# LouisRouss/DiffuLab

Hardware: AMD Instinct MI355X
Metric: train images/sec/node (DiT-S/2 flow-matching, 256x256 latents) (higher is better)
Workload: dtype bf16

## Files before the change

diffulab_amd/csrc/attention.hip:

```cpp
#include "common.h"
#include "attn_paths.h"

static std::atomic<int> g_last_attn_path{DL_ATTN_PATH_NONE};
void dl_note_attn_path(int path) { g_last_attn_path.store(path, std::memory_order_relaxed); }
extern "C" __attribute__((visibility("default"))) int dl_lab_last_attn_path() { return g_last_attn_path.load(std::memory_order_relaxed); }

typedef __attribute__((address_space(3))) void lds_void_t;
typedef const __attribute__((address_space(1))) void glb_void_t;

#define DH 64
#define ROWB 128
#define LOG2E 1.4426950408889634f
#define LN2 0.6931471805599453f

__device__ __forceinline__ int swz8(int row) {
  const int v = (row >> 1) & 7;
  return ((v & 1) << 2) | (v >> 1);
}
__device__ __forceinline__ int tile_off(int row, int slot) { return row * ROWB + ((slot ^ swz8(row)) << 4); }

__device__ __forceinline__ void tile_dma(const bf16_t* __restrict__ g, int64_t pitch, char* tile, int nrows, int wave,
                                         int nwaves, int lane) {
  const int nchunk = nrows >> 3;
  for (int c = wave; c < nchunk; c += nwaves) {
// ... 576 lines not shown
    f32x16_t s[2];
#pragma unroll
    for (int t = 0; t < 2; ++t) {
#pragma unroll
      for (int r = 0; r < 16; ++r) s[t][r] = 0.f;
#pragma unroll
      for (int ks = 0; ks < 4; ++ks) s[t] = MFMA(frag_rows(kt, kb + t * 32 + (lane & 31), ks, hi), qf[ks], s[t]);
    }
    float mx = -INFINITY;
#pragma unroll
    for (int t = 0; t < 2; ++t)
#pragma unroll
      for (int r = 0; r < 16; ++r) {
        s[t][r] *= c;
        mx = fmaxf(mx, s[t][r]);
      }
    mx = fmaxf(mx, __shfl_xor(mx, 32, 64));
    const float m_new = fmaxf(m_run, mx);
    const float alpha = fast_exp2(m_run - m_new);
    m_run = m_new;
    float ps = 0.f;
    float p[2][16];
#pragma unroll
    for (int t = 0; t < 2; ++t)
#pragma unroll
      for (int r = 0; r < 16; ++r) {
        p[t][r] = fast_exp2(s[t][r] - m_new);
        ps += p[t][r];
      }
    l_run = l_run * alpha + ps;
#pragma unroll
    for (int r = 0; r < 16; ++r) {
      o[0][r] *= alpha;
      o[1][r] *= alpha;
    }
#pragma unroll
    for (int t = 0; t < 2; ++t)
#pragma unroll
      for (int kg2 = 0; kg2 < 2; ++kg2) {
        const bf16x8_t pf = pack_frag(&p[t][kg2 * 8]);
        const int rbase = kb + t * 32 + kg2 * 16;
        o[0] = MFMA(frag_cols(vt, rbase, 0, lane), pf, o[0]);
        o[1] = MFMA(frag_cols(vt, rbase, 32, lane), pf, o[1]);
      }
  }
  const float l_tot = l_run + __shfl_xor(l_run, 32, 64);
  const float inv = 1.0f / l_tot;
  store_rows64(out + ((int64_t)b * N + qrow) * (H * DH) + h * DH, o, inv, hi);
  if (hi == 0) lse[(int64_t)bh * N + qrow] = (m_run + log2f(l_tot)) * LN2;
}

static int g_attn_pipe = 1;
extern "C" __attribute__((visibility("default"))) void dl_lab_set_attn_pipe(int mode) { g_attn_pipe = mode; }
static int attn_fwd_pipe_on() { return g_attn_pipe & 1; }
#define PIPE_N 256
__global__ __launch_bounds__(512) void attn_fwd_qkn_pipe_k(const bf16_t* __restrict__ qkv, bf16_t* __restrict__ out, float* __restrict__ lse,
                                                           int H, int items, float scale, QkNorm qn) {
  constexpr int N = PIPE_N;
  extern __shared__ __attribute__((aligned(16))) char smem[];
  const int lane = threadIdx.x & 63, hi = lane >> 5, l31 = lane & 31;
  const int wave = __builtin_amdgcn_readfirstlane(threadIdx.x >> 6);
  const int per = (items + (int)gridDim.x - 1) / (int)gridDim.x;
  const int it0 = blockIdx.x * per, it1 = it0 + per < items ? it0 + per : items;
  if (it0 >= it1) return;
  const int D = H * DH, half = qn.rot >> 1;
  const int qrow = wave * 32 + l31;
  f32x4_t qc[4], qs[4];
#pragma unroll
  for (int ks = 0; ks < 4; ++ks) {
    const int d0 = ks * 16 + hi * 8;
    if (d0 < qn.rot) {
      qc[ks] = *(const f32x4_t*)(qn.cs + (int64_t)qrow * half + (d0 >> 1));
      qs[ks] = *(const f32x4_t*)(qn.sn + (int64_t)qrow * half + (d0 >> 1));
    } else {
      qc[ks] = qs[ks] = f32x4_t{0.f, 0.f, 0.f, 0.f};
    }
  }
  int ro[4];
#pragma unroll
  for (int ks = 0; ks < 4; ++ks) ro[ks] = tile_off(l31, ks * 2 + hi);
  int co[2][2];
  {
    const int li = lane & 15, g = lane >> 4;
#pragma unroll
    for (int cb = 0; cb < 2; ++cb)
#pragma unroll
      for (int hh = 0; hh < 2; ++hh) {
        const int col = cb * 32 + (g & 1) * 16 + (li & 3) * 4, r = (g >> 1) * 4 + (li >> 2) + 8 * hh;
        co[cb][hh] = r * ROWB + (((col >> 3) ^ swz8(r)) << 4) + (col & 7) * 2;
      }
  }
  const float c = scale * LOG2E;
  float* sq_l = (float*)(smem + 4 * N * ROWB);
  float* sk_l = sq_l + D;
  for (int i = threadIdx.x; i < D; i += blockDim.x) {
    sq_l[i] = qn.sq[i];
    sk_l[i] = qn.sk[i];
  }

  u32x4_t qraw[4];
  float ssq_q, ssq_k;
  u32x4_t opk[4];
  float lse_pend = 0.f;
  auto store_pending = [&](int item) {
    const int b = item / H, h = item - b * H;
    bf16_t* rowp = out + ((int64_t)b * N + qrow) * (H * DH) + h * DH;
#pragma unroll
    for (int dt = 0; dt < 2; ++dt)
#pragma unroll
      for (int gp = 0; gp < 2; ++gp) *(u32x4_t*)(rowp + dt * 32 + 16 * gp + 8 * hi) = opk[dt * 2 + gp];
    if (hi == 0) lse[(int64_t)item * N + qrow] = lse_pend;
  };
  auto issue_tiles = [&](int item, int buf) {
    const int b = item / H, h = item - b * H;
    const bf16_t* base = qkv + (int64_t)b * N * qn.pitch + h * DH;
    char* kt = smem + buf * (2 * N * ROWB);
    tile_dma(base + D, qn.pitch, kt, N, wave, 8, lane);
    tile_dma(base + 2 * D, qn.pitch, kt + N * ROWB, N, wave, 8, lane);
  };
  auto issue_regs = [&](int item) {
    const int b = item / H, h = item - b * H;
    const bf16_t* base = qkv + (int64_t)b * N * qn.pitch + h * DH;
#pragma unroll
    for (int ks = 0; ks < 4; ++ks) qraw[ks] = *(const u32x4_t*)(base + (int64_t)qrow * qn.pitch + ks * 16 + hi * 8);
    const float2 sq2 = *(const float2*)(qn.ssq + ((int64_t)b * N + qrow) * 2);
    ssq_q = sq2.x;
    ssq_k = sq2.y;
  };
  issue_regs(it0);
  issue_tiles(it0, 0);

  for (int it = it0; it < it1; ++it) {
    const int buf = (it - it0) & 1;
    char* kt = smem + buf * (2 * N * ROWB);
    char* vt = kt + N * ROWB;
    const int b = it / H, h = it - b * H, bh = it;
    const int64_t tok = (int64_t)b * N + qrow;
    asm volatile("s_waitcnt vmcnt(0)" ::: "memory");
    __syncthreads();
    const float rq = rsqrtf(ssq_q * qn.inv_d + qn.eps);
    bf16x8_t qf[4];
#pragma unroll
    for (int ks = 0; ks < 4; ++ks) {
      const int d0 = ks * 16 + hi * 8;
      const u32x4_t t = qk_xform8(qraw[ks], rq, sq_l + h * DH + d0, (const float*)&qc[ks], (const float*)&qs[ks], d0 < qn.rot);
      qf[ks] = __builtin_bit_cast(bf16x8_t, t);
      if (qn.qo) *(u32x4_t*)(qn.qo + ((int64_t)bh * N + qrow) * DH + d0) = t;
    }
    if (qn.rrms && h == 0 && hi == 0) qn.rrms[tok * 2] = rq;
    const float rk = rsqrtf(ssq_k * qn.inv_d + qn.eps);
#pragma unroll
    for (int ks = 0; ks < 4; ++ks) {
      const int d0 = ks * 16 + hi * 8;
      char* p = kt + wave * 32 * ROWB + ro[ks];
      const u32x4_t t = qk_xform8(*(const u32x4_t*)p, rk, sk_l + h * DH + d0, (const float*)&qc[ks], (const float*)&qs[ks], d0 < qn.rot);
      *(u32x4_t*)p = t;
      if (qn.ko) *(u32x4_t*)(qn.ko + ((int64_t)bh * N + qrow) * DH + d0) = t;
    }
    if (qn.rrms && h == 0 && hi == 0) qn.rrms[tok * 2 + 1] = rk;
    if (it > it0) store_pending(it - 1);
    if (it + 1 < it1) issue_regs(it + 1);
    __syncthreads();
    if (it + 1 < it1) issue_tiles(it + 1, buf ^ 1);

    f32x16_t o[2];
#pragma unroll
    for (int r = 0; r < 16; ++r) o[0][r] = o[1][r] = 0.f;
    float m_run = -INFINITY, l_run = 0.f;
#pragma unroll 1
    for (int kb = 0; kb < N; kb += 64) {
      union {
        s16x4_t h[2];
        bf16x8_t v;
      } vf[2][2][2];
#pragma unroll
      for (int t = 0; t < 2; ++t)
#pragma unroll
        for (int kg2 = 0; kg2 < 2; ++kg2)
#pragma unroll
          for (int cb = 0; cb < 2; ++cb) {
            const char* pb = vt + (kb + t * 32 + kg2 * 16) * ROWB;
            vf[t][kg2][cb].h[0] = attn_lds_tr16(pb + co[cb][0]);
            vf[t][kg2][cb].h[1] = attn_lds_tr16(pb + co[cb][1]);
          }
      f32x16_t s[2];
#pragma unroll
      for (int t = 0; t < 2; ++t) {
#pragma unroll
        for (int r = 0; r < 16; ++r) s[t][r] = 0.f;
#pragma unroll
        for (int ks = 0; ks < 4; ++ks) s[t] = MFMA(*(const bf16x8_t*)(kt + (kb + t * 32) * ROWB + ro[ks]), qf[ks], s[t]);
      }
      float mx = -INFINITY;
#pragma unroll
      for (int t = 0; t < 2; ++t)
#pragma unroll
        for (int r = 0; r < 16; ++r) {
          s[t][r] *= c;
          mx = fmaxf(mx, s[t][r]);
        }
      mx = fmaxf(mx, __shfl_xor(mx, 32, 64));
      const float m_new = fmaxf(m_run, mx);
      const float alpha = fast_exp2(m_run - m_new);
      m_run = m_new;
      float ps = 0.f;
      float p[2][16];
#pragma unroll
      for (int t = 0; t < 2; ++t)
#pragma unroll
        for (int r = 0; r < 16; ++r) {
          p[t][r] = fast_exp2(s[t][r] - m_new);
          ps += p[t][r];
        }
      l_run = l_run * alpha + ps;
#pragma unroll
      for (int r = 0; r < 16; ++r) {
        o[0][r] *= alpha;
        o[1][r] *= alpha;
      }
      asm volatile("s_waitcnt lgkmcnt(0)" ::: "memory");
#pragma unroll
      for (int t = 0; t < 2; ++t)
#pragma unroll
        for (int kg2 = 0; kg2 < 2; ++kg2)
#pragma unroll
          for (int cb = 0; cb < 2; ++cb) asm volatile("" : "+v"(vf[t][kg2][cb].v));
#pragma unroll
      for (int t = 0; t < 2; ++t)
#pragma unroll
        for (int kg2 = 0; kg2 < 2; ++kg2) {
          const bf16x8_t pf = pack_frag(&p[t][kg2 * 8]);
          o[0] = MFMA(vf[t][kg2][0].v, pf, o[0]);
          o[1] = MFMA(vf[t][kg2][1].v, pf, o[1]);
        }
    }
    const float l_tot = l_run + __shfl_xor(l_run, 32, 64);
    const float inv = 1.0f / l_tot;
    pack_rows64(opk, o, inv);
    lse_pend = (m_run + log2f(l_tot)) * LN2;
  }
  store_pending(it1 - 1);
}

extern "C" int dl_attn_fwd_qkn(const void* qkv, const float* ssq, const float* scale_q, const float* scale_k, const float* cos,
                               const float* sin, float eps, int64_t rot, void* q_out, void* k_out, float* rrms, void* out, float* lse,
                               int64_t B, int64_t H, int64_t N, int64_t dh, float scale, dl_stream_t stream) {
  DL_CHECK_ARG(qkv && ssq && scale_q && scale_k && out && lse && B > 0 && H > 0, "dl_attn_fwd_qkn: null operand");
  DL_CHECK_ARG((q_out && k_out && rrms) || (!q_out && !k_out && !rrms), "dl_attn_fwd_qkn: q_out, k_out and rrms are kept together (training) or not at all");
  DL_CHECK_ARG(rot == 0 || (cos && sin), "dl_attn_fwd_qkn: rot > 0 needs the cos / sin tables");
  DL_CHECK_ARG(dh == DH && rot % 8 == 0 && rot <= DH, "dl_attn_fwd_qkn: head_dim 64, rot %% 8 == 0 (dh=%lld rot=%lld)", (long long)dh,
               (long long)rot);
  DL_CHECK_ARG(N % 64 == 0 && N >= 64 && N <= 256, "dl_attn_fwd_qkn: N=%lld must be a multiple of 64 up to 256", (long long)N);
  DL_CHECK_ARG((((uintptr_t)qkv | (uintptr_t)q_out | (uintptr_t)k_out | (uintptr_t)out | (uintptr_t)scale_q | (uintptr_t)scale_k |
                 (uintptr_t)cos | (uintptr_t)sin) & 15) == 0, "dl_attn_fwd_qkn: 16-byte alignment");
  const int lds = (int)(2 * N * ROWB);
  static DevOnce once;
  (void)dev_cus(once, [] { (void)hipFuncSetAttribute((const void*)attn_fwd_qkn_k, hipFuncAttributeMaxDynamicSharedMemorySize, 2 * 256 * ROWB); });
  const int64_t D = H * DH;
  QkNorm qn{ssq, scale_q, scale_k, cos, sin, (bf16_t*)q_out, (bf16_t*)k_out, rrms, 1.0f / (float)D, eps, (int)rot, (int)(3 * D)};
  const int cus = dev_cus(once, [] {});
  if (N == PIPE_N && D <= 2048 && B * H >= 3 * (int64_t)cus && attn_fwd_pipe_on()) {
    static DevOnce once2;
    (void)dev_cus(once2, [] { (void)hipFuncSetAttribute((const void*)attn_fwd_qkn_pipe_k, hipFuncAttributeMaxDynamicSharedMemorySize, 4 * PIPE_N * ROWB + 8 * 2048); });
    const int items = (int)(B * H);
    const int per = (items + cus - 1) / cus, grid = (items + per - 1) / per;
    dl_note_attn_path(ATTN_FWD_QKN_PIPE);
    hipLaunchKernelGGL(attn_fwd_qkn_pipe_k, grid, 512, 4 * PIPE_N * ROWB + 8 * (int)D, (hipStream_t)stream, (const bf16_t*)qkv, (bf16_t*)out, lse, (int)H,
                       items, scale, qn);
    DL_LAUNCH_CHECK();
    return DL_OK;
  }
  dl_note_attn_path(ATTN_FWD_QKN_CHAIN);
  hipLaunchKernelGGL(attn_fwd_qkn_k, (int)(B * H), (int)(N / 32) * 64, lds, (hipStream_t)stream, (const bf16_t*)qkv, (bf16_t*)out, lse, (int)H,
                     (int)N, scale, qn);
  DL_LAUNCH_CHECK();
  return DL_OK;
}

__device__ __forceinline__ bf16x8_t frag_rows_g(const bf16_t* __restrict__ g, int64_t pitch, int row, int ks, int hi) {
  return *(const bf16x8_t*)(g + (int64_t)row * pitch + (ks * 2 + hi) * 8);
}

__global__ __launch_bounds__(256, 2) void attn_bwd_k(const bf16_t* __restrict__ q, const bf16_t* __restrict__ k,
                                                     const bf16_t* __restrict__ v, const bf16_t* __restrict__ out,
                                                     const bf16_t* __restrict__ dout, const float* __restrict__ lse,
                                                     bf16_t* __restrict__ dq, bf16_t* __restrict__ dk,
                                                     bf16_t* __restrict__ dv, int H, int N, float scale, HeadLayout vl,
                                                     HeadLayout dvl, HeadLayout dql) {
  extern __shared__ __attribute__((aligned(16))) char smem[];
  char* ta = smem;
  char* tb = ta + N * ROWB;
  float* lse2 = (float*)(tb + N * ROWB);
  float* delta = lse2 + N;
  const int lane = threadIdx.x & 63, hi = lane >> 5;
  const int wave = __builtin_amdgcn_readfirstlane(threadIdx.x >> 6), nwaves = blockDim.x >> 6;
  const int bh = blockIdx.x, b = bh / H, h = bh - b * H;
  const int64_t hoff = (int64_t)bh * N * DH;
  const int64_t tok_pitch = (int64_t)H * DH;
  const bf16_t* og = out + (int64_t)b * N * tok_pitch + h * DH;
  const bf16_t* dog = dout + (int64_t)b * N * tok_pitch + h * DH;
  tile_dma(k + hoff, DH, ta, N, wave, nwaves, lane);
  const bf16_t* vg = v + b * vl.bs + h * vl.hs;
  tile_dma(vg, vl.pitch, tb, N, wave, nwaves, lane);
  asm volatile("s_waitcnt vmcnt(0)" ::: "memory");
  __syncthreads();

  const float c = scale * LOG2E;

  for (int ob = 0; ob < 2; ++ob) {
    const int own = (wave * 2 + ob) * 32;
    bf16x8_t qf[4], dof[4];
#pragma unroll
    for (int ks = 0; ks < 4; ++ks) {
      qf[ks] = frag_rows_g(q + hoff, DH, own + (lane & 31), ks, hi);
      dof[ks] = frag_rows_g(dog, tok_pitch, own + (lane & 31), ks, hi);
    }
    float my_delta = 0.f;
#pragma unroll
    for (int ks = 0; ks < 4; ++ks) {
      const bf16x8_t of = frag_rows_g(og, tok_pitch, own + (lane & 31), ks, hi);
#pragma unroll
      for (int e = 0; e < 8; ++e) my_delta += (float)of[e] * (float)dof[ks][e];
    }
    my_delta += __shfl_xor(my_delta, 32, 64);
    const float my_lse = lse[(int64_t)bh * N + own + (lane & 31)] * LOG2E;
    if (hi == 0) {
      delta[own + (lane & 31)] = my_delta;
      lse2[own + (lane & 31)] = my_lse;
    }
    f32x16_t dqa[2];
#pragma unroll
    for (int r = 0; r < 16; ++r) dqa[0][r] = dqa[1][r] = 0.f;
    auto scores = [&](int kb, f32x16_t& st, f32x16_t& dpt) {
#pragma unroll
      for (int r = 0; r < 16; ++r) st[r] = dpt[r] = 0.f;
#pragma unroll
      for (int ks = 0; ks < 4; ++ks) {
        st = MFMA(frag_rows(ta, kb + (lane & 31), ks, hi), qf[ks], st);
        dpt = MFMA(frag_rows(tb, kb + (lane & 31), ks, hi), dof[ks], dpt);
      }
    };
    auto step = [&](int kb, f32x16_t& st, f32x16_t& dpt, f32x16_t& stn, f32x16_t& dptn) {
      if (kb + 32 < N) scores(kb + 32, stn, dptn);
      float ds[16];
#pragma unroll
      for (int r = 0; r < 16; ++r) {
        const float p = fast_exp2(st[r] * c - my_lse);
        ds[r] = p * (dpt[r] - my_delta);
      }
#pragma unroll
      for (int kg2 = 0; kg2 < 2; ++kg2) {
        const bf16x8_t df = pack_frag(&ds[kg2 * 8]);
        dqa[0] = MFMA(frag_cols(ta, kb + kg2 * 16, 0, lane), df, dqa[0]);
        dqa[1] = MFMA(frag_cols(ta, kb + kg2 * 16, 32, lane), df, dqa[1]);
      }
    };
    f32x16_t s0, d0, s1, d1;
    scores(0, s0, d0);
    for (int kb = 0; kb < N; kb += 64) {
      step(kb, s0, d0, s1, d1);
      step(kb + 32, s1, d1, s0, d0);
    }
    store_rows64(dq + b * dql.bs + h * dql.hs + (int64_t)(own + (lane & 31)) * dql.pitch, dqa, scale, hi);
  }

  __syncthreads();
  tile_dma(q + hoff, DH, ta, N, wave, nwaves, lane);
  tile_dma(dog, tok_pitch, tb, N, wave, nwaves, lane);
  asm volatile("s_waitcnt vmcnt(0)" ::: "memory");
  __syncthreads();

  for (int ob = 0; ob < 2; ++ob) {
    const int own = (wave * 2 + ob) * 32;
    bf16x8_t kf[4], vf[4];
#pragma unroll
    for (int ks = 0; ks < 4; ++ks) {
      kf[ks] = frag_rows_g(k + hoff, DH, own + (lane & 31), ks, hi);
      vf[ks] = frag_rows_g(vg, vl.pitch, own + (lane & 31), ks, hi);
    }
    f32x16_t dka[2], dva[2];
#pragma unroll
    for (int r = 0; r < 16; ++r) dka[0][r] = dka[1][r] = dva[0][r] = dva[1][r] = 0.f;
    auto scores_t = [&](int qb, f32x16_t& s) {
#pragma unroll
      for (int r = 0; r < 16; ++r) s[r] = 0.f;
#pragma unroll
      for (int ks = 0; ks < 4; ++ks) s = MFMA(frag_rows(ta, qb + (lane & 31), ks, hi), kf[ks], s);
    };
    auto step_t = [&](int qb, f32x16_t& s, f32x16_t& sn) {
      f32x16_t dp;
#pragma unroll
      for (int r = 0; r < 16; ++r) dp[r] = 0.f;
#pragma unroll
      for (int ks = 0; ks < 4; ++ks) dp = MFMA(frag_rows(tb, qb + (lane & 31), ks, hi), vf[ks], dp);
      if (qb + 32 < N) scores_t(qb + 32, sn);
      float p[16], ds[16];
#pragma unroll
      for (int g4 = 0; g4 < 4; ++g4) {
        const f32x4_t l4 = *(const f32x4_t*)(lse2 + qb + g4 * 8 + hi * 4);
        const f32x4_t d4 = *(const f32x4_t*)(delta + qb + g4 * 8 + hi * 4);
#pragma unroll
        for (int e = 0; e < 4; ++e) {
          const int r = g4 * 4 + e;
          p[r] = fast_exp2(s[r] * c - l4[e]);
          ds[r] = p[r] * (dp[r] - d4[e]);
        }
      }
#pragma unroll
      for (int kg2 = 0; kg2 < 2; ++kg2) {
        const bf16x8_t pf = pack_frag(&p[kg2 * 8]);
        const bf16x8_t df = pack_frag(&ds[kg2 * 8]);
        const int rbase = qb + kg2 * 16;
        dva[0] = MFMA(frag_cols(tb, rbase, 0, lane), pf, dva[0]);
        dva[1] = MFMA(frag_cols(tb, rbase, 32, lane), pf, dva[1]);
        dka[0] = MFMA(frag_cols(ta, rbase, 0, lane), df, dka[0]);
        dka[1] = MFMA(frag_cols(ta, rbase, 32, lane), df, dka[1]);
      }
    };
    f32x16_t s0, s1;
    scores_t(0, s0);
    for (int qb = 0; qb < N; qb += 32) {
      step_t(qb, s0, s1);
      s0 = s1;
    }
    store_rows64(dk + b * dql.bs + h * dql.hs + (int64_t)(own + (lane & 31)) * dql.pitch, dka, scale, hi);
    store_rows64(dv + b * dvl.bs + h * dvl.hs + (int64_t)(own + (lane & 31)) * dvl.pitch, dva, 1.0f, hi);
  }
}

__global__ __launch_bounds__(256, 2) void attn_bwd_tiled_k(const bf16_t* __restrict__ q, const bf16_t* __restrict__ k,
                                                           const bf16_t* __restrict__ v, const bf16_t* __restrict__ out,
                                                           const bf16_t* __restrict__ dout, const float* __restrict__ lse,
                                                           bf16_t* __restrict__ dq, bf16_t* __restrict__ dk,
                                                           bf16_t* __restrict__ dv, int H, int Nq, int Nk, float scale,
                                                           const float* __restrict__ key_bias) {
  extern __shared__ __attribute__((aligned(16))) char smem[];
  char* ta = smem;
  char* tb = ta + ACH * ROWB;
  float* lse2 = (float*)(tb + ACH * ROWB);
  float* delta = lse2 + Nq;
  float* bs = delta + Nq;
  const int lane = threadIdx.x & 63, hi = lane >> 5;
  const int wave = __builtin_amdgcn_readfirstlane(threadIdx.x >> 6), nwaves = blockDim.x >> 6;
  const int nchq = Nq / ACH, nchk = Nk / ACH, nmax = nchq > nchk ? nchq : nchk;
  const int bh = blockIdx.x / nmax, cc = blockIdx.x - bh * nmax, b = bh / H, h = bh - b * H;
  const int64_t hoffq = (int64_t)bh * Nq * DH, hoffk = (int64_t)bh * Nk * DH;
  const int64_t tok_pitch = (int64_t)H * DH;
  const bf16_t* og = out + (int64_t)b * Nq * tok_pitch + h * DH;
  const bf16_t* dog = dout + (int64_t)b * Nq * tok_pitch + h * DH;
  for (int row = threadIdx.x >> 1; row < Nq; row += blockDim.x >> 1) {
    const int half = threadIdx.x & 1;
    const bf16_t* po = og + (int64_t)row * tok_pitch + half * 32;
    const bf16_t* pd = dog + (int64_t)row * tok_pitch + half * 32;
    float acc = 0.f;
#pragma unroll
    for (int i = 0; i < 4; ++i) {
      float a[8], d[8];
      unpack8(*(const u32x4_t*)(po + i * 8), a);
      unpack8(*(const u32x4_t*)(pd + i * 8), d);
#pragma unroll
      for (int e = 0; e < 8; ++e) acc += a[e] * d[e];
    }
    acc += __shfl_xor(acc, 1, 64);
    if (half == 0) {
      delta[row] = acc;
      lse2[row] = lse[(int64_t)bh * Nq + row] * LOG2E;
    }
  }
  const float c = scale * LOG2E;

  if (cc < nchq) {
    bf16x8_t qf[2][4], dof[2][4];
    float my_lse[2], my_delta[2];
    f32x16_t dqa[2][2];
#pragma unroll
    for (int ob = 0; ob < 2; ++ob) {
      const int own = cc * ACH + (wave * 2 + ob) * 32;
#pragma unroll
      for (int ks = 0; ks < 4; ++ks) {
        qf[ob][ks] = frag_rows_g(q + hoffq, DH, own + (lane & 31), ks, hi);
        dof[ob][ks] = frag_rows_g(dog, tok_pitch, own + (lane & 31), ks, hi);
      }
#pragma unroll
      for (int r = 0; r < 16; ++r) dqa[ob][0][r] = dqa[ob][1][r] = 0.f;
    }
    for (int kc = 0; kc < nchk; ++kc) {
      __syncthreads();
      tile_dma(k + hoffk + (int64_t)kc * ACH * DH, DH, ta, ACH, wave, nwaves, lane);
      tile_dma(v + hoffk + (int64_t)kc * ACH * DH, DH, tb, ACH, wave, nwaves, lane);
      for (int i = threadIdx.x; i < ACH; i += blockDim.x)
        bs[i] = key_bias ? key_bias[(int64_t)b * Nk + kc * ACH + i] * LOG2E : 0.f;
      asm volatile("s_waitcnt vmcnt(0)" ::: "memory");
      __syncthreads();
      if (kc == 0) {
#pragma unroll
        for (int ob = 0; ob < 2; ++ob) {
          const int own = cc * ACH + (wave * 2 + ob) * 32;
          my_lse[ob] = lse2[own + (lane & 31)];
          my_delta[ob] = delta[own + (lane & 31)];
        }
      }
#pragma unroll
      for (int ob = 0; ob < 2; ++ob)
        for (int kb = 0; kb < ACH; kb += 32) {
          f32x16_t st, dpt;
#pragma unroll
          for (int r = 0; r < 16; ++r) st[r] = dpt[r] = 0.f;
#pragma unroll
          for (int ks = 0; ks < 4; ++ks) {
            st = MFMA(frag_rows(ta, kb + (lane & 31), ks, hi), qf[ob][ks], st);
            dpt = MFMA(frag_rows(tb, kb + (lane & 31), ks, hi), dof[ob][ks], dpt);
          }
          float ds[16];
#pragma unroll
          for (int g4 = 0; g4 < 4; ++g4) {
            const f32x4_t b4 = *(const f32x4_t*)(bs + kb + g4 * 8 + hi * 4);
#pragma unroll
            for (int e = 0; e < 4; ++e) {
              const int r = g4 * 4 + e;
              const float p = fast_exp2(st[r] * c + b4[e] - my_lse[ob]);
              ds[r] = p * (dpt[r] - my_delta[ob]);
            }
          }
#pragma unroll
          for (int kg2 = 0; kg2 < 2; ++kg2) {
            const bf16x8_t df = pack_frag(&ds[kg2 * 8]);
            dqa[ob][0] = MFMA(frag_cols(ta, kb + kg2 * 16, 0, lane), df, dqa[ob][0]);
            dqa[ob][1] = MFMA(frag_cols(ta, kb + kg2 * 16, 32, lane), df, dqa[ob][1]);
          }
        }
    }
#pragma unroll
    for (int ob = 0; ob < 2; ++ob) {
      const int own = cc * ACH + (wave * 2 + ob) * 32;
      store_rows64(dq + hoffq + (int64_t)(own + (lane & 31)) * DH, dqa[ob], scale, hi);
    }
  }

  for (int ob = 0; ob < 2 && cc < nchk; ++ob) {
    const int own = cc * ACH + (wave * 2 + ob) * 32;
    const float kbias = key_bias ? key_bias[(int64_t)b * Nk + own + (lane & 31)] * LOG2E : 0.f;
    bf16x8_t kf[4], vf[4];
#pragma unroll
    for (int ks = 0; ks < 4; ++ks) {
      kf[ks] = frag_rows_g(k + hoffk, DH, own + (lane & 31), ks, hi);
      vf[ks] = frag_rows_g(v + hoffk, DH, own + (lane & 31), ks, hi);
    }
    f32x16_t dka[2], dva[2];
#pragma unroll
    for (int r = 0; r < 16; ++r) dka[0][r] = dka[1][r] = dva[0][r] = dva[1][r] = 0.f;
    for (int qc = 0; qc < nchq; ++qc) {
      __syncthreads();
      tile_dma(q + hoffq + (int64_t)qc * ACH * DH, DH, ta, ACH, wave, nwaves, lane);
      tile_dma(dog + (int64_t)qc * ACH * tok_pitch, tok_pitch, tb, ACH, wave, nwaves, lane);
      asm volatile("s_waitcnt vmcnt(0)" ::: "memory");
      __syncthreads();
      for (int qb = 0; qb < ACH; qb += 32) {
        f32x16_t s2, dp;
#pragma unroll
        for (int r = 0; r < 16; ++r) s2[r] = dp[r] = 0.f;
#pragma unroll
        for (int ks = 0; ks < 4; ++ks) {
          s2 = MFMA(frag_rows(ta, qb + (lane & 31), ks, hi), kf[ks], s2);
          dp = MFMA(frag_rows(tb, qb + (lane & 31), ks, hi), vf[ks], dp);
        }
        float p[16], ds[16];
#pragma unroll
        for (int g4 = 0; g4 < 4; ++g4) {
          const f32x4_t l4 = *(const f32x4_t*)(lse2 + qc * ACH + qb + g4 * 8 + hi * 4);
          const f32x4_t d4 = *(const f32x4_t*)(delta + qc * ACH + qb + g4 * 8 + hi * 4);
#pragma unroll
          for (int e = 0; e < 4; ++e) {
            const int r = g4 * 4 + e;
            p[r] = fast_exp2(s2[r] * c + kbias - l4[e]);
            ds[r] = p[r] * (dp[r] - d4[e]);
          }
        }
#pragma unroll
        for (int kg2 = 0; kg2 < 2; ++kg2) {
          const bf16x8_t pf = pack_frag(&p[kg2 * 8]);
          const bf16x8_t df = pack_frag(&ds[kg2 * 8]);
          const int rbase = qb + kg2 * 16;
          dva[0] = MFMA(frag_cols(tb, rbase, 0, lane), pf, dva[0]);
          dva[1] = MFMA(frag_cols(tb, rbase, 32, lane), pf, dva[1]);
          dka[0] = MFMA(frag_cols(ta, rbase, 0, lane), df, dka[0]);
          dka[1] = MFMA(frag_cols(ta, rbase, 32, lane), df, dka[1]);
        }
      }
    }
    store_rows64(dk + hoffk + (int64_t)(own + (lane & 31)) * DH, dka, scale, hi);
    store_rows64(dv + hoffk + (int64_t)(own + (lane & 31)) * DH, dva, 1.0f, hi);
  }
}

__device__ __forceinline__ const float* delta_row(const bf16_t* dq_head, int row) {
  return (const float*)(dq_head + (int64_t)(row & ~31) * DH) + (row & 31);
}
__global__ __launch_bounds__(256) void attn_bwd_delta_k(const bf16_t* __restrict__ out, const bf16_t* __restrict__ dout,
                                                        bf16_t* __restrict__ dq, int H, int Nq) {
  const int64_t pr = (int64_t)blockIdx.x * 128 + (threadIdx.x >> 1);
  const int half = threadIdx.x & 1;
  const int h = (int)(pr % H);
  const int64_t bn = pr / H;
  const int n = (int)(bn % Nq), b = (int)(bn / Nq);
  const bf16_t* po = out + pr * DH + half * 32;
  const bf16_t* pd = dout + pr * DH + half * 32;
  float acc = 0.f;
#pragma unroll
  for (int i = 0; i < 4; ++i) {
    float a[8], d[8];
    unpack8(*(const u32x4_t*)(po + i * 8), a);
    unpack8(*(const u32x4_t*)(pd + i * 8), d);
#pragma unroll
    for (int e = 0; e < 8; ++e) acc += a[e] * d[e];
  }
  acc += __shfl_xor(acc, 1, 64);
  if (half == 0) *(float*)delta_row(dq + ((int64_t)b * H + h) * Nq * DH, n) = acc;
}

__global__ __launch_bounds__(256, 2) void attn_bwd_dkdv_long_k(const bf16_t* __restrict__ q, const bf16_t* __restrict__ k,
                                                               const bf16_t* __restrict__ v, const bf16_t* __restrict__ dout,
                                                               const float* __restrict__ lse, const bf16_t* __restrict__ dq,
                                                               bf16_t* __restrict__ dk, bf16_t* __restrict__ dv, int H, int Nq, int Nk,
                                                               float scale, const float* __restrict__ key_bias) {
  extern __shared__ __attribute__((aligned(16))) char smem[];
  char* ta = smem;
  char* tb = ta + ACH * ROWB;
  float* lse2 = (float*)(tb + ACH * ROWB);
  float* delta = lse2 + ACH;
  const int lane = threadIdx.x & 63, hi = lane >> 5;
  const int wave = __builtin_amdgcn_readfirstlane(threadIdx.x >> 6), nwaves = blockDim.x >> 6;
  const int nchq = Nq / ACH, nchk = Nk / ACH;
  const int bh = blockIdx.x / nchk, cc = blockIdx.x - bh * nchk, b = bh / H, h = bh - b * H;
  const int64_t hoffq = (int64_t)bh * Nq * DH, hoffk = (int64_t)bh * Nk * DH;
  const int64_t tok_pitch = (int64_t)H * DH;
  const bf16_t* dog = dout + (int64_t)b * Nq * tok_pitch + h * DH;
  const float c = scale * LOG2E;
  for (int ob = 0; ob < 2; ++ob) {
    const int own = cc * ACH + (wave * 2 + ob) * 32;
    const float kbias = key_bias ? key_bias[(int64_t)b * Nk + own + (lane & 31)] * LOG2E : 0.f;
    bf16x8_t kf[4], vf[4];
#pragma unroll
    for (int ks = 0; ks < 4; ++ks) {
      kf[ks] = frag_rows_g(k + hoffk, DH, own + (lane & 31), ks, hi);
      vf[ks] = frag_rows_g(v + hoffk, DH, own + (lane & 31), ks, hi);
    }
    f32x16_t dka[2], dva[2];
#pragma unroll
    for (int r = 0; r < 16; ++r) dka[0][r] = dka[1][r] = dva[0][r] = dva[1][r] = 0.f;
    for (int qc = 0; qc < nchq; ++qc) {
      __syncthreads();
      tile_dma(q + hoffq + (int64_t)qc * ACH * DH, DH, ta, ACH, wave, nwaves, lane);
      tile_dma(dog + (int64_t)qc * ACH * tok_pitch, tok_pitch, tb, ACH, wave, nwaves, lane);
      for (int i = threadIdx.x; i < ACH; i += blockDim.x) {
        lse2[i] = lse[(int64_t)bh * Nq + qc * ACH + i] * LOG2E;
        delta[i] = *delta_row(dq + hoffq, qc * ACH + i);
      }
      asm volatile("s_waitcnt vmcnt(0)" ::: "memory");
      __syncthreads();
      for (int qb = 0; qb < ACH; qb += 32) {
        f32x16_t s2, dp;
#pragma unroll
        for (int r = 0; r < 16; ++r) s2[r] = dp[r] = 0.f;
#pragma unroll
        for (int ks = 0; ks < 4; ++ks) {
          s2 = MFMA(frag_rows(ta, qb + (lane & 31), ks, hi), kf[ks], s2);
          dp = MFMA(frag_rows(tb, qb + (lane & 31), ks, hi), vf[ks], dp);
        }
        float p[16], ds[16];
#pragma unroll
        for (int g4 = 0; g4 < 4; ++g4) {
          const f32x4_t l4 = *(const f32x4_t*)(lse2 + qb + g4 * 8 + hi * 4);
          const f32x4_t d4 = *(const f32x4_t*)(delta + qb + g4 * 8 + hi * 4);
#pragma unroll
          for (int e = 0; e < 4; ++e) {
            const int r = g4 * 4 + e;
            p[r] = fast_exp2(s2[r] * c + kbias - l4[e]);
            ds[r] = p[r] * (dp[r] - d4[e]);
          }
        }
#pragma unroll
        for (int kg2 = 0; kg2 < 2; ++kg2) {
          const bf16x8_t pf = pack_frag(&p[kg2 * 8]);
          const bf16x8_t df = pack_frag(&ds[kg2 * 8]);
          const int rbase = qb + kg2 * 16;
          dva[0] = MFMA(frag_cols(tb, rbase, 0, lane), pf, dva[0]);
          dva[1] = MFMA(frag_cols(tb, rbase, 32, lane), pf, dva[1]);
          dka[0] = MFMA(frag_cols(ta, rbase, 0, lane), df, dka[0]);
          dka[1] = MFMA(frag_cols(ta, rbase, 32, lane), df, dka[1]);
        }
      }
    }
    store_rows64(dk + hoffk + (int64_t)(own + (lane & 31)) * DH, dka, scale, hi);
    store_rows64(dv + hoffk + (int64_t)(own + (lane & 31)) * DH, dva, 1.0f, hi);
  }
}

__global__ __launch_bounds__(256, 2) void attn_bwd_dq_long_k(const bf16_t* __restrict__ q, const bf16_t* __restrict__ k,
                                                             const bf16_t* __restrict__ v, const bf16_t* __restrict__ dout,
                                                             const float* __restrict__ lse, bf16_t* __restrict__ dq, int H, int Nq,
                                                             int Nk, float scale, const float* __restrict__ key_bias) {
  extern __shared__ __attribute__((aligned(16))) char smem[];
  char* ta = smem;
  char* tb = ta + ACH * ROWB;
  float* bs = (float*)(tb + ACH * ROWB);
  const int lane = threadIdx.x & 63, hi = lane >> 5;
  const int wave = __builtin_amdgcn_readfirstlane(threadIdx.x >> 6), nwaves = blockDim.x >> 6;
  const int nchq = Nq / ACH, nchk = Nk / ACH;
  const int bh = blockIdx.x / nchq, cc = blockIdx.x - bh * nchq, b = bh / H, h = bh - b * H;
  const int64_t hoffq = (int64_t)bh * Nq * DH, hoffk = (int64_t)bh * Nk * DH;
  const int64_t tok_pitch = (int64_t)H * DH;
  const bf16_t* dog = dout + (int64_t)b * Nq * tok_pitch + h * DH;
  const float c = scale * LOG2E;
  bf16x8_t qf[2][4], dof[2][4];
  float my_lse[2], my_delta[2];
  f32x16_t dqa[2][2];
#pragma unroll
  for (int ob = 0; ob < 2; ++ob) {
    const int own = cc * ACH + (wave * 2 + ob) * 32;
#pragma unroll
    for (int ks = 0; ks < 4; ++ks) {
      qf[ob][ks] = frag_rows_g(q + hoffq, DH, own + (lane & 31), ks, hi);
      dof[ob][ks] = frag_rows_g(dog, tok_pitch, own + (lane & 31), ks, hi);
    }
    my_lse[ob] = lse[(int64_t)bh * Nq + own + (lane & 31)] * LOG2E;
    my_delta[ob] = *delta_row(dq + hoffq, own + (lane & 31));
#pragma unroll
    for (int r = 0; r < 16; ++r) dqa[ob][0][r] = dqa[ob][1][r] = 0.f;
  }
// ... 575 lines not shown
```

Baseline: 12750.

## Keep owned Q/dO/O fragments in registers and rebuild LDS tiles from registers

The fused attention backward kernel now loads each wave's own Q, dO and O fragments and LSE once, overlapping the first load with the K/V tile DMA. It then writes Q and dO into the LDS tiles from those registers instead of re-reading the full tiles from global memory. K/V fragments for the dK/dV phase are taken from LDS rather than re-fetched from global. This removes redundant global traffic and the second DMA wait, at the cost of more live registers (doubled fragment arrays, both ob loops unrolled), which may raise register pressure or reduce occupancy.

```diff
diff --git a/diffulab_amd/csrc/attention.hip b/diffulab_amd/csrc/attention.hip
--- a/diffulab_amd/csrc/attention.hip
+++ b/diffulab_amd/csrc/attention.hip
@@ -902,28 +902,36 @@
   tile_dma(k + hoff, DH, ta, N, wave, nwaves, lane);
   const bf16_t* vg = v + b * vl.bs + h * vl.hs;
   tile_dma(vg, vl.pitch, tb, N, wave, nwaves, lane);
+  bf16x8_t qf[2][4], dof[2][4], of[2][4];
+  float lse_own[2];
+  auto load_own = [&](int ob) {
+    const int row = (wave * 2 + ob) * 32 + (lane & 31);
+#pragma unroll
+    for (int ks = 0; ks < 4; ++ks) {
+      qf[ob][ks] = frag_rows_g(q + hoff, DH, row, ks, hi);
+      dof[ob][ks] = frag_rows_g(dog, tok_pitch, row, ks, hi);
+      of[ob][ks] = frag_rows_g(og, tok_pitch, row, ks, hi);
+    }
+    lse_own[ob] = lse[(int64_t)bh * N + row];
+  };
+  load_own(0);
   asm volatile("s_waitcnt vmcnt(0)" ::: "memory");
   __syncthreads();
+  load_own(1);
 
   const float c = scale * LOG2E;
 
+#pragma unroll
   for (int ob = 0; ob < 2; ++ob) {
     const int own = (wave * 2 + ob) * 32;
-    bf16x8_t qf[4], dof[4];
+    float my_delta = 0.f;
 #pragma unroll
     for (int ks = 0; ks < 4; ++ks) {
-      qf[ks] = frag_rows_g(q + hoff, DH, own + (lane & 31), ks, hi);
-      dof[ks] = frag_rows_g(dog, tok_pitch, own + (lane & 31), ks, hi);
-    }
-    float my_delta = 0.f;
-#pragma unroll
-    for (int ks = 0; ks < 4; ++ks) {
-      const bf16x8_t of = frag_rows_g(og, tok_pitch, own + (lane & 31), ks, hi);
-#pragma unroll
-      for (int e = 0; e < 8; ++e) my_delta += (float)of[e] * (float)dof[ks][e];
+#pragma unroll
+      for (int e = 0; e < 8; ++e) my_delta += (float)of[ob][ks][e] * (float)dof[ob][ks][e];
     }
     my_delta += __shfl_xor(my_delta, 32, 64);
-    const float my_lse = lse[(int64_t)bh * N + own + (lane & 31)] * LOG2E;
+    const float my_lse = lse_own[ob] * LOG2E;
     if (hi == 0) {
       delta[own + (lane & 31)] = my_delta;
       lse2[own + (lane & 31)] = my_lse;
@@ -936,8 +944,8 @@
       for (int r = 0; r < 16; ++r) st[r] = dpt[r] = 0.f;
 #pragma unroll
       for (int ks = 0; ks < 4; ++ks) {
-        st = MFMA(frag_rows(ta, kb + (lane & 31), ks, hi), qf[ks], st);
-        dpt = MFMA(frag_rows(tb, kb + (lane & 31), ks, hi), dof[ks], dpt);
+        st = MFMA(frag_rows(ta, kb + (lane & 31), ks, hi), qf[ob][ks], st);
+        dpt = MFMA(frag_rows(tb, kb + (lane & 31), ks, hi), dof[ob][ks], dpt);
       }
     };
     auto step = [&](int kb, f32x16_t& st, f32x16_t& dpt, f32x16_t& stn, f32x16_t& dptn) {
@@ -964,20 +972,29 @@
     store_rows64(dq + b * dql.bs + h * dql.hs + (int64_t)(own + (lane & 31)) * dql.pitch, dqa, scale, hi);
   }
 
+  bf16x8_t kf[2][4], vf[2][4];
+#pragma unroll
+  for (int ob = 0; ob < 2; ++ob)
+#pragma unroll
+    for (int ks = 0; ks < 4; ++ks) {
+      kf[ob][ks] = frag_rows(ta, (wave * 2 + ob) * 32 + (lane & 31), ks, hi);
+      vf[ob][ks] = frag_rows(tb, (wave * 2 + ob) * 32 + (lane & 31), ks, hi);
+    }
+  asm volatile("s_waitcnt lgkmcnt(0)" ::: "memory");
   __syncthreads();
-  tile_dma(q + hoff, DH, ta, N, wave, nwaves, lane);
-  tile_dma(dog, tok_pitch, tb, N, wave, nwaves, lane);
-  asm volatile("s_waitcnt vmcnt(0)" ::: "memory");
+#pragma unroll
+  for (int ob = 0; ob < 2; ++ob)
+#pragma unroll
+    for (int ks = 0; ks < 4; ++ks) {
+      const int off = tile_off((wave * 2 + ob) * 32 + (lane & 31), ks * 2 + hi);
+      *(bf16x8_t*)(ta + off) = qf[ob][ks];
+      *(bf16x8_t*)(tb + off) = dof[ob][ks];
+    }
   __syncthreads();
 
+#pragma unroll
   for (int ob = 0; ob < 2; ++ob) {
     const int own = (wave * 2 + ob) * 32;
-    bf16x8_t kf[4], vf[4];
-#pragma unroll
-    for (int ks = 0; ks < 4; ++ks) {
-      kf[ks] = frag_rows_g(k + hoff, DH, own + (lane & 31), ks, hi);
-      vf[ks] = frag_rows_g(vg, vl.pitch, own + (lane & 31), ks, hi);
-    }
     f32x16_t dka[2], dva[2];
 #pragma unroll
     for (int r = 0; r < 16; ++r) dka[0][r] = dka[1][r] = dva[0][r] = dva[1][r] = 0.f;
@@ -985,14 +1002,14 @@
 #pragma unroll
       for (int r = 0; r < 16; ++r) s[r] = 0.f;
 #pragma unroll
-      for (int ks = 0; ks < 4; ++ks) s = MFMA(frag_rows(ta, qb + (lane & 31), ks, hi), kf[ks], s);
+      for (int ks = 0; ks < 4; ++ks) s = MFMA(frag_rows(ta, qb + (lane & 31), ks, hi), kf[ob][ks], s);
     };
     auto step_t = [&](int qb, f32x16_t& s, f32x16_t& sn) {
       f32x16_t dp;
 #pragma unroll
       for (int r = 0; r < 16; ++r) dp[r] = 0.f;
 #pragma unroll
-      for (int ks = 0; ks < 4; ++ks) dp = MFMA(frag_rows(tb, qb + (lane & 31), ks, hi), vf[ks], dp);
+      for (int ks = 0; ks < 4; ++ks) dp = MFMA(frag_rows(tb, qb + (lane & 31), ks, hi), vf[ob][ks], dp);
       if (qb + 32 < N) scores_t(qb + 32, sn);
       float p[16], ds[16];
 #pragma unroll
@@ -1023,8 +1040,10 @@
       step_t(qb, s0, s1);
       s0 = s1;
     }
-    store_rows64(dk + b * dql.bs + h * dql.hs + (int64_t)(own + (lane & 31)) * dql.pitch, dka, scale, hi);
-    store_rows64(dv + b * dvl.bs + h * dvl.hs + (int64_t)(own + (lane & 31)) * dvl.pitch, dva, 1.0f, hi);
+    int row = own + (lane & 31);
+    asm volatile("" : "+v"(row));
+    store_rows64(dk + b * dql.bs + h * dql.hs + (int64_t)row * dql.pitch, dka, scale, hi);
+    store_rows64(dv + b * dvl.bs + h * dvl.hs + (int64_t)row * dvl.pitch, dva, 1.0f, hi);
   }
 }
 
```

Result: no change. 12840, median of 6 (+0.7%).
